# mantasu/face-crop-plus

Hardware: AMD Instinct MI355X
Metric: faces/sec end-to-end (detect+align+crop) (higher is better)
Workload: dtype f16x3; 1 GPU; RetinaFace detect + 5-pt align/crop, batch=32/GPU synthetic 1024x1024 RGB, strategy=largest, det_threshold=0.6, output 256x256, detector on 2 HIP streams x 16 images; global_batch=32, image_size=1024, parallelism=dp1

## Files before the change

### face-crop-plus_amd/csrc/fcp_bneck_chain.hip

```cpp
#include "fcp_conv_common.h"

#include <type_traits>

using namespace fcp_conv;

namespace {

constexpr int FCP_CHAIN_STORE_AUX = 2;

struct ChainK {
  const float* t1;  unsigned t1_bytes;  int t1_ld;
  const float* w2;  unsigned w2_bytes;  const float* ws2;  const float* b2;
  const float* w3;  unsigned w3_bytes;  const float* ws3;  const float* b3;
  const float* res; int res_ld;
  float* out;       int out_ld;    unsigned out_bytes;
  const float* w1n; unsigned w1n_bytes; const float* ws1n; const float* b1n;
  float* t1n;       int t1n_ld;
  int n, h, w, M;
  int nt_store;
  int out_even;
  const float* t1b; unsigned t1b_bytes; int t1b_ld, hb, wb, sb;
};

constexpr int BMT = 128;
constexpr int C = 64;
constexpr int ROWB = 128;
constexpr int STAGE = (BMT + C) * ROWB;
constexpr int CT_OFF = 0;
constexpr int W1B_OFF = BMT * 128;
constexpr bool w1_double(int cn, bool has_c2) { return !has_c2 || W1B_OFF + 2 * cn * 128 + 2 * C * 128 <= 2 * STAGE; }
constexpr int w3b_off(int cn, bool has_c2) { return W1B_OFF + (w1_double(cn, has_c2) ? 2 : 1) * cn * 128; }
constexpr int r0_bytes(int cw, int cn, bool has_c2) { return has_c2 ? 2 * STAGE : w3b_off(cn, has_c2) + 2 * cw * 128; }
constexpr bool alias_t2(bool has_c2) { return !has_c2; }
constexpr int lds_bytes(int cw, int cn, bool has_c2, bool direct = false) {
  const int r0 = r0_bytes(cw, cn, has_c2), t2 = BMT * cw * 4;
  if (direct) return r0;
  return !alias_t2(has_c2) ? r0 + t2 : (r0 > W1B_OFF + t2 ? r0 : W1B_OFF + t2);
}
constexpr int wgs_per_cu(int cw, int cn, bool has_c2, bool direct = false) {
  if (direct) return cn == 0 && lds_bytes(cw, cn, has_c2, true) <= 80 * 1024 ? 2 : 1;
  return lds_bytes(cw, cn, has_c2) <= 80 * 1024 ? 2 : 1;
}

__device__ __forceinline__ void mfma3(f32x16& acc, const f16x8& ah, const f16x8& al, const f16x8& bh, const f16x8& bl) {
  acc = __builtin_amdgcn_mfma_f32_32x32x16_f16(al, bh, acc, 0, 0, 0);
  acc = __builtin_amdgcn_mfma_f32_32x32x16_f16(ah, bl, acc, 0, 0, 0);
  acc = __builtin_amdgcn_mfma_f32_32x32x16_f16(ah, bh, acc, 0, 0, 0);
}

__device__ __forceinline__ void row_values8(const float* c8, const float (&ws8)[8], const float (&b8)[8], float (&v)[8]) {
  const f32x4 a = *reinterpret_cast<const f32x4*>(c8);
  const f32x4 b = *reinterpret_cast<const f32x4*>(c8 + 4);
#pragma unroll
  for (int e = 0; e < 4; ++e) {
    v[e] = conv_value_relu(a[e], ws8[e], b8[e]);
    v[4 + e] = conv_value_relu(b[e], ws8[4 + e], b8[4 + e]);
  }
}

constexpr bool direct_form(int cn, int cw2) { return cw2 > 0 || cn == 0; }
template <int CN, int CW, int NOUT, bool HAS_C2, bool HAS_RES, int CW2 = 0>
__global__ void __launch_bounds__(2 * BMT, wgs_per_cu(CW, CN, HAS_C2, direct_form(CN, CW2))) bneck_chain_c64(const ChainK p) {
  constexpr bool DIRECT = direct_form(CN, CW2);
  static_assert(!DIRECT || (!HAS_C2 && CW2 % 32 == 0 && CW2 < CW), "direct forms are pair forms");
  constexpr bool HAS_P3 = CN > 0;
  static_assert(!HAS_C2 || CW == C, "phase 1 is written for 64-channel bottlenecks");
  constexpr bool PATCH = HAS_C2;
  constexpr int PH = BMT / 16;
  constexpr int NTHR = 2 * BMT;
  constexpr int NW = NTHR / 64;
  constexpr int LR = NTHR / 8;
  constexpr int TN3 = CN / 32;
  constexpr int TN3A = TN3 > 0 ? TN3 : 1;
  constexpr int CS = CW / 32;
  constexpr int NCH = NOUT / 32;
  constexpr int W3CH = CW * 128;
  constexpr bool ALIAS = alias_t2(HAS_C2) && !DIRECT;
  constexpr int T2_OFF = ALIAS ? W1B_OFF : r0_bytes(CW, CN, HAS_C2);
  constexpr int WGS = wgs_per_cu(CW, CN, HAS_C2, DIRECT);
  constexpr int WPS = WGS * NW / 4;
  static_assert(lds_bytes(CW, CN, HAS_C2, DIRECT) <= 160 * 1024, "LDS budget");
  constexpr bool W1DB = w1_double(CN, HAS_C2);
  constexpr bool SPREAD = W1DB && (HAS_C2 || WPS == 1);
  constexpr bool W1PRE = W1DB && !DIRECT && (HAS_C2 ? CN <= 64 || WPS == 1 : CN <= 128 && WPS == 1);
  constexpr int W3B_OFF = w3b_off(CN, HAS_C2);
  static_assert(!HAS_C2 || W3B_OFF + 2 * W3CH <= 2 * STAGE, "chunk buffers must fit the phase-1 stage region");
  constexpr int NRES = HAS_RES ? 4 : 0;
  extern __shared__ __attribute__((aligned(16))) float smem[];
  char* lds = reinterpret_cast<char*>(smem);

  const int tile_m = xcd_tile_order(gridDim.x, blockIdx.x);

  const int tid = threadIdx.x;
  const int lane = tid & 63;
  const int wave = tid >> 6;
  const int wave_u = __builtin_amdgcn_readfirstlane(wave);
  const int lrow = tid >> 3;
  const int csrc = (tid & 7) ^ swz(lrow);
  const int l31 = lane & 31, half = lane >> 5;
  int offH[2], offL[2];
  frag_offsets(lane, offH, offL);
  auto frag_pair = [&](const char* row, int s, f16x8& hi, f16x8& lo) {
    hi = *reinterpret_cast<const f16x8*>(row + offH[s]);
    lo = *reinterpret_cast<const f16x8*>(row + offL[s]);
  };
  const int hw = p.h * p.w;
  int pn = 0, py0 = 0, px0 = 0;
  if constexpr (PATCH) {
    const int txn = (p.w + 15) >> 4, tyn = (p.h + PH - 1) / PH;
    const int r = tile_m / txn;
    px0 = (tile_m - r * txn) * 16;
    pn = r / tyn;
    py0 = (r - pn * tyn) * PH;
  }
  auto pix = [&](int row) -> long {
    if constexpr (PATCH) {
      const int y = py0 + (row >> 4), x = px0 + (row & 15);
      return (y < p.h && x < p.w) ? ((long)pn * p.h + y) * p.w + x : -1L;
    } else {
// ... 6 lines not shown
    float* Cs = smem;
#pragma unroll
    for (int i = 0; i < 2; ++i)
#pragma unroll
      for (int rr = 0; rr < 16; ++rr) {
        const int row = wm * 64 + i * 32 + (rr & 3) + 8 * (rr >> 2) + 4 * half;
        Cs[row * C + wn * 32 + l31] = acc1[i][rr];
      }
    __syncthreads();
    {
      const int ccol = (tid & 7) * 8;
      float ws8[8], b8[8];
#pragma unroll
      for (int e = 0; e < 8; ++e) {
        ws8[e] = p.ws2[ccol + e];
        b8[e] = p.b2[ccol + e];
      }
#pragma unroll
      for (int g = 0; g < 4; ++g) {
        const int row = (tid >> 3) + LR * g;
        float v[8];
        row_values8(Cs + row * C + ccol, ws8, b8, v);
        u32x4_t hi, lo;
        split8(f32x4{v[0], v[1], v[2], v[3]}, f32x4{v[4], v[5], v[6], v[7]}, hi, lo);
        const int q = (ccol & 31) >> 3, sw = swz(row);
        char* trow = lds + T2_OFF + (ccol >> 5) * (BMT * ROWB) + row * ROWB;
        *reinterpret_cast<u32x4_t*>(trow + ((q ^ sw) << 4)) = hi;
        *reinterpret_cast<u32x4_t*>(trow + (((4 + q) ^ sw) << 4)) = lo;
      }
    }
    __syncthreads();
  };

  if constexpr (HAS_C2) {
    constexpr int HALO = (PH + 2) * 18;
    constexpr int HROWS = (HALO + LR - 1) / LR * LR;
    constexpr int ASL = HROWS * ROWB;
    constexpr int TPB = 2, NSTEP = 18 / TPB;
    static_assert(18 % TPB == 0, "taps per barrier must divide the 18 K slices");
    constexpr int BST_OFF = 2 * ASL, BSL = C * ROWB, BSTG = TPB * BSL;
    static_assert(BST_OFF + 2 * BSTG <= T2_OFF + BMT * C * 4, "halo patch + filter stages must fit region 0 + T2");
    f32x16 acc1[2];
    const int wm = wave / 2, wn = wave % 2;
    __amdgpu_buffer_rsrc_t rs_in = __builtin_amdgcn_make_buffer_rsrc(const_cast<float*>(p.t1), 0, p.t1_bytes, 0x00020000);
    __amdgpu_buffer_rsrc_t rs_w = __builtin_amdgcn_make_buffer_rsrc(const_cast<float*>(p.w2), 0, p.w2_bytes, 0x00020000);
#pragma unroll
    for (int i = 0; i < HROWS / LR; ++i) {
      const int r = lrow + LR * i;
      const int hy = r / 18, hx = r - hy * 18;
      const int y = py0 - 1 + hy, x = px0 - 1 + hx;
      const bool ok = r < HALO && (unsigned)y < (unsigned)p.h && (unsigned)x < (unsigned)p.w;
      const unsigned src = ok ? ((unsigned)((pn * p.h + y) * p.w + x) * (unsigned)p.t1_ld + (unsigned)(csrc * 4)) * 4u : 0xFFFFFFFFu;
#pragma unroll
      for (int cs = 0; cs < 2; ++cs)
        __builtin_amdgcn_raw_ptr_buffer_load_lds(rs_in, (__attribute__((address_space(3))) void*)(lds + cs * ASL + (wave_u * 8 + LR * i) * ROWB), 16,
                                                 (int)(src == 0xFFFFFFFFu ? 0xFFFFFFFFu : src + (unsigned)(cs * 32 * 4)), 0, 0, 0);
    }
    constexpr int B_LD = C / LR;
    unsigned woff[B_LD];
#pragma unroll
    for (int i = 0; i < B_LD; ++i) woff[i] = (unsigned)(((lrow + LR * i) * (9 * C) + csrc * 4) * 4);
    auto dma_b = [&](int step, int stage) {
#pragma unroll
      for (int u = 0; u < TPB; ++u)
#pragma unroll
        for (int i = 0; i < B_LD; ++i)
          __builtin_amdgcn_raw_ptr_buffer_load_lds(rs_w, (__attribute__((address_space(3))) void*)(lds + BST_OFF + stage * BSTG + u * BSL + (wave_u * 8 + LR * i) * ROWB), 16,
                                                   (int)(woff[i] + (unsigned)((step * TPB + u) * BK * 4)), 0, 0, 0);
    };
    dma_b(0, 0);
#pragma unroll
    for (int i = 0; i < 2; ++i)
#pragma unroll
      for (int e = 0; e < 16; ++e) acc1[i][e] = 0.f;
    int hr0[2];
#pragma unroll
    for (int i = 0; i < 2; ++i) hr0[i] = (wm * 4 + i * 2 + (l31 >> 4)) * 18 + (l31 & 15);
    const char* Bw = lds + BST_OFF + (wn * 32 + l31) * ROWB;
    fcp_static_for<0, NSTEP>([&](auto gc) {
      constexpr int g = decltype(gc)::value;
      asm volatile("s_waitcnt vmcnt(0)" ::: "memory");
      __builtin_amdgcn_s_barrier();
      __builtin_amdgcn_sched_barrier(0);
      fcp_static_for<0, TPB>([&](auto uc) {
        constexpr int kt = g * TPB + decltype(uc)::value, cs = kt / 9, tap = kt % 9;
        const char* Bb = Bw + (g & 1) * BSTG + decltype(uc)::value * BSL;
        f16x8 ah[2][2], al[2][2], bh[2], bl[2];
#pragma unroll
        for (int i = 0; i < 2; ++i) {
          const int hr = hr0[i] + (tap / 3) * 18 + tap % 3;
          const int sw = swz(hr);
          const char* Ab = lds + cs * ASL + hr * ROWB;
#pragma unroll
          for (int sq = 0; sq < 2; ++sq) {
            ah[sq][i] = *reinterpret_cast<const f16x8*>(Ab + (((2 * sq + half) ^ sw) << 4));
            al[sq][i] = *reinterpret_cast<const f16x8*>(Ab + (((4 + 2 * sq + half) ^ sw) << 4));
          }
        }
#pragma unroll
        for (int sq = 0; sq < 2; ++sq) {
          frag_pair(Bb, sq, bh[sq], bl[sq]);
        }
        if constexpr (decltype(uc)::value == TPB - 1) {
// ... 67 lines not shown

  const char* a2base = lds + T2_OFF + (wave * 32 + l31) * ROWB;
  const char* a3base = lds + CT_OFF + (wave * 32 + l31) * ROWB;
  const int eq = lane & 3;
  const int erow0 = wave * 32 + (lane >> 2);
  long rm[2];
  unsigned so[2];
#pragma unroll
  for (int it = 0; it < 2; ++it) {
    const int prow = erow0 + 16 * it;
    const long m = pix(prow);
    rm[it] = m >= 0 ? m : (long)p.M - 1;
    const bool keep = !PATCH || !p.out_even || ((((prow >> 4) | prow) & 1) == 0);
    so[it] = (m >= 0 && keep) ? (unsigned)(m * p.out_ld * 4 + eq * 16) : 0xFFFFFFFFu;
  }
  __amdgpu_buffer_rsrc_t rs_out = __builtin_amdgcn_make_buffer_rsrc(p.out, 0, p.out_bytes, 0x00020000);

  u32x4_t rhi[2], rlo[2];
  auto load_res = [&](int j) {
    if constexpr (!HAS_RES) return;
#pragma unroll
    for (int it = 0; it < 2; ++it) {
      const char* pb = reinterpret_cast<const char*>(p.res) + rm[it] * p.res_ld * 4 + j * 128 + eq * 16;
      rhi[it] = *reinterpret_cast<const u32x4_t*>(pb);
      rlo[it] = *reinterpret_cast<const u32x4_t*>(pb + 64);
    }
  };
  const int nch = NCH;
  float ws_l = p.ws3[l31], b_l = p.b3[l31];
  constexpr int NCONST = 2;
  f16x8 ah[CS][2], al[CS][2];
  auto read_a2 = [&]() {
#pragma unroll
    for (int sl = 0; sl < CS; ++sl)
#pragma unroll
      for (int s = 0; s < 2; ++s) {
        frag_pair(a2base + sl * BMT * ROWB, s, ah[sl][s], al[sl][s]);
      }
  };
  if constexpr (DIRECT) {
    constexpr int CS1 = (CW - CW2) / 32;
    __amdgpu_buffer_rsrc_t rs_a = __builtin_amdgcn_make_buffer_rsrc(const_cast<float*>(p.t1), 0, p.t1_bytes, 0x00020000);
    __amdgpu_buffer_rsrc_t rs_b = __builtin_amdgcn_make_buffer_rsrc(const_cast<float*>(p.t1b), 0, p.t1b_bytes, 0x00020000);
    asm volatile("" ::: "memory");
    dma_w3(0, 0);
    if constexpr (W1DB) dma_w1(0, 0);
    asm volatile("" ::: "memory");
    const long m = pix(wave * 32 + l31);
    unsigned oa = 0xFFFFFFFFu, ob = 0xFFFFFFFFu;
    if (m >= 0) {
      const int ni = (int)(m / hw);
      const int rem = (int)(m - (long)ni * hw);
      const int y = rem / p.w, x = rem - y * p.w;
      oa = (unsigned)m * (unsigned)p.t1_ld * 4u;
      ob = ((unsigned)(ni * p.hb + y * p.sb) * (unsigned)p.wb + (unsigned)(x * p.sb)) * (unsigned)p.t1b_ld * 4u;
    }
#pragma unroll
    for (int sl = 0; sl < CS; ++sl)
#pragma unroll
      for (int sk = 0; sk < 2; ++sk) {
        const bool first = sl < CS1;
        const unsigned base = first ? oa : ob;
        const unsigned off = (unsigned)((first ? sl : sl - CS1) * 128);
        const unsigned vh = base == 0xFFFFFFFFu ? base : base + off + (unsigned)((2 * sk + half) << 4);
        const unsigned vl = base == 0xFFFFFFFFu ? base : base + off + (unsigned)((4 + 2 * sk + half) << 4);
        ah[sl][sk] = __builtin_bit_cast(f16x8, __builtin_amdgcn_raw_buffer_load_b128(first ? rs_a : rs_b, (int)vh, 0, 0));
        al[sl][sk] = __builtin_bit_cast(f16x8, __builtin_amdgcn_raw_buffer_load_b128(first ? rs_a : rs_b, (int)vl, 0, 0));
      }
    asm volatile("s_waitcnt vmcnt(0)" ::: "memory");
#pragma unroll
    for (int sl = 0; sl < CS; ++sl)
#pragma unroll
      for (int sk = 0; sk < 2; ++sk) asm volatile("" : "+v"(ah[sl][sk]), "+v"(al[sl][sk]));
    __builtin_amdgcn_sched_barrier(0);
  }
  if constexpr (ALIAS) {
    asm volatile("s_waitcnt vmcnt(0)" ::: "memory");
    __builtin_amdgcn_s_barrier();
    __builtin_amdgcn_sched_barrier(0);
    read_a2();
    asm volatile("s_waitcnt lgkmcnt(0)" ::: "memory");
    __builtin_amdgcn_s_barrier();
    __builtin_amdgcn_sched_barrier(0);
  }
  asm volatile("" ::: "memory");
  if constexpr (!DIRECT) {
    dma_w3(0, 0);
    if constexpr (W1DB) dma_w1(0, 0);
  }
  asm volatile("" ::: "memory");
  if (nch > 0) load_res(0);
  __builtin_amdgcn_sched_barrier(0);

  for (int j = 0; j < nch; ++j) {
    const bool more = j + 1 < NCH;
    if (j == 0) asm volatile("s_waitcnt vmcnt(%0)" ::"n"(NRES) : "memory");
    else asm volatile("s_waitcnt vmcnt(%0)" ::"n"(4 + NCONST + NRES) : "memory");
    asm volatile("s_waitcnt lgkmcnt(0)" ::: "memory");
    __builtin_amdgcn_s_barrier();
    __builtin_amdgcn_sched_barrier(0);
    if constexpr (!SPREAD) {
      if (more) dma_w3(j + 1, (j + 1) & 1);
      if constexpr (W1DB) {
        if (more) dma_w1(j + 1, (j + 1) & 1);
      } else {
        dma_w1(j, 0);
      }
    }
    asm volatile("" ::: "memory");
    __builtin_amdgcn_sched_barrier(0);
    const char* b2base = lds + W3B_OFF + (j & 1) * W3CH + l31 * ROWB;
    if constexpr (!ALIAS && !DIRECT) {
      if (j == 0) read_a2();
    }
    constexpr int BG = (CS <= 4 && (HAS_C2 || WPS == 1)) ? CS : 2;
    f16x8 bh[2][BG][2], bl[2][BG][2];
    auto read_b2 = [&](int buf, int g) {
#pragma unroll
      for (int q = 0; q < BG; ++q)
#pragma unroll
        for (int s = 0; s < 2; ++s) {
          frag_pair(b2base + (g * BG + q) * 4096, s, bh[buf][q][s], bl[buf][q][s]);
        }
    };
    read_b2(0, 0);
    f16x8 dh[2][TN3A], dl[2][TN3A];
    if constexpr (W1PRE) {
      const char* w1b = lds + W1B_OFF + (j & 1) * (CN * ROWB);
#pragma unroll
      for (int s = 0; s < 2; ++s)
#pragma unroll
        for (int t = 0; t < TN3; ++t) {
          frag_pair(w1b + (t * 32 + l31) * ROWB, s, dh[s][t], dl[s][t]);
        }
      __builtin_amdgcn_sched_barrier(0);
    }
    f32x16 acc2;
#pragma unroll
    for (int e = 0; e < 16; ++e) acc2[e] = 0.f;
    fcp_static_for<0, CS / BG>([&](auto gc) {
      constexpr int g = decltype(gc)::value;
      if constexpr (g + 1 < CS / BG) read_b2((g + 1) & 1, g + 1);
      fcp_static_for<0, 2 * BG>([&](auto tc) {
        constexpr int q = decltype(tc)::value / 2, s = decltype(tc)::value % 2, sl = g * BG + q, trip = 2 * sl + s;
        mfma3(acc2, ah[sl][s], al[sl][s], bh[g & 1][q][s], bl[g & 1][q][s]);
        constexpr int PER = (NDMA + 2 * CS - 1) / (2 * CS);
        if constexpr (SPREAD && trip * PER < NDMA) {
          __builtin_amdgcn_sched_barrier(0);
// ... 99 lines not shown
#pragma unroll
  for (int hh = 0; hh < CN / 64; ++hh) {
#pragma unroll
    for (int t = 0; t < 2; ++t)
#pragma unroll
      for (int rr = 0; rr < 16; ++rr) {
        const int row = wave * 32 + (rr & 3) + 8 * (rr >> 2) + 4 * half;
        Cs[row * 64 + t * 32 + l31] = acc3[CN == 64 ? t : 2 * hh + t][rr];
      }
    __syncthreads();
    const int ccol = (tid & 7) * 8;
    const int co = hh * 64 + ccol;
    float ws8[8], b8[8];
#pragma unroll
    for (int e = 0; e < 8; ++e) {
      ws8[e] = p.ws1n[co + e];
      b8[e] = p.b1n[co + e];
    }
#pragma unroll
    for (int g = 0; g < 4; ++g) {
      const int row = (tid >> 3) + LR * g;
      const long m = pix(row);
      if (m < 0) continue;
      float v[8];
      row_values8(Cs + row * 64 + ccol, ws8, b8, v);
      pack_store8(p.t1n, m, p.t1n_ld, co, 1, p.nt_store, v);
    }
    __syncthreads();
  }
}

template <int CN, int CW, int NOUT, bool HAS_C2, bool HAS_RES, int CW2 = 0>
int launch(const ChainK& k, hipStream_t s) {
  constexpr int LDS = lds_bytes(CW, CN, HAS_C2, direct_form(CN, CW2));
  FCP_LDS_OPT_IN((&bneck_chain_c64<CN, CW, NOUT, HAS_C2, HAS_RES, CW2>), LDS);
  const int tiles = HAS_C2 ? k.n * fcp_cdiv(k.h, BMT / 16) * ((k.w + 15) >> 4) : fcp_cdiv(k.M, BMT);
  hipLaunchKernelGGL((bneck_chain_c64<CN, CW, NOUT, HAS_C2, HAS_RES, CW2>), dim3(tiles), dim3(2 * BMT), LDS, s, k);
  FCP_LAUNCH_OK();
  return 0;
}

struct ChainForm {
  bool has_c2;
  int c, cb, nout;
  bool residual;
  int cn;
  int (*launch)(const ChainK&, hipStream_t);
};
const ChainForm FORMS[] = {
    {true, 64, 0, 256, true, 64, launch<64, 64, 256, true, true>},
    {true, 64, 0, 256, true, 128, launch<128, 64, 256, true, true>},
    {false, 128, 0, 512, true, 128, launch<128, 128, 512, false, true>},
    {false, 128, 0, 256, false, 64, launch<64, 128, 256, false, false>},
    {false, 256, 0, 1024, true, 256, launch<256, 256, 1024, false, true>},
    {false, 128, 0, 512, true, 256, launch<256, 128, 512, false, true>},
    {false, 384, 256, 512, false, 128, launch<128, 384, 512, false, false, 256>},
    {false, 256, 0, 1024, true, 0, launch<0, 256, 1024, false, true>},
};

}

extern "C" int fcp_bottleneck_chain_f16x3(const fcp_chain_desc* d, fcp_stream_t stream) {
  FCP_REQUIRE(d != nullptr, "chain: null descriptor");
  const bool has_p3 = d->cn != 0 || d->w1n != nullptr;
  FCP_REQUIRE(d->t1 && d->w3 && d->ws3 && d->b3 && d->out && (!has_p3 || (d->w1n && d->ws1n && d->b1n && d->t1n)),
              "chain: null pointer (every convolution carries folded-BN bias and filter scales)");
  const bool has_c2 = d->w2 != nullptr;
  FCP_REQUIRE(!has_c2 || (d->ws2 && d->b2), "chain: conv2 needs its scales and bias");
  const int cb = d->t1b ? d->cb : 0;
  const ChainForm* form = nullptr;
  for (const ChainForm& f : FORMS)
    if (f.has_c2 == has_c2 && f.c == d->c && f.cb == cb && f.nout == d->nout && f.residual == (d->res != nullptr) && f.cn == d->cn &&
        (f.cn != 0) == has_p3)
      form = &f;
  FCP_REQUIRE((form && form->cb) || !d->t1b, "chain: a second source (t1b) exists for the two-source pair form only (c 384 = 128 + 256, nout 512, cn 128)");
  FCP_REQUIRE(form != nullptr, "chain: unsupported shape (c %d, conv2 %d, nout %d, residual %d, cn %d)", d->c, (int)has_c2, d->nout,
              d->res != nullptr, d->cn);
  FCP_REQUIRE(d->n > 0 && d->h > 0 && d->w > 0, "chain: bad sizes");
  const long M = (long)d->n * d->h * d->w;
  FCP_REQUIRE(M < (1L << 31), "chain: too many pixels");
  auto aligned = [](const void* p, int ld) { return ((uintptr_t)p & 127) == 0 && ld % 32 == 0; };
  FCP_REQUIRE(aligned(d->t1, d->t1_ld) && (!d->res || aligned(d->res, d->res_ld)) && aligned(d->out, d->out_ld) && (!has_p3 || aligned(d->t1n, d->t1n_ld)),
              "chain: tensors are split32 views: 128-byte aligned, channel stride a multiple of 32");
  FCP_REQUIRE(d->t1_ld >= d->c - cb && (!d->res || d->res_ld >= d->nout) && d->out_ld >= d->nout && (!has_p3 || d->t1n_ld >= d->cn), "chain: channel strides too small");
  const unsigned long t1_bytes = (unsigned long)M * d->t1_ld * 4ul;
  FCP_REQUIRE(t1_bytes < 0xFFFFFFF0ul, "chain: t1 must be below 4 GiB");
  ChainK k;
  k.t1 = d->t1; k.t1_bytes = (unsigned)t1_bytes; k.t1_ld = d->t1_ld;
  k.w2 = reinterpret_cast<const float*>(d->w2); k.w2_bytes = 128u * 9 * 64 * 4; k.ws2 = d->ws2; k.b2 = d->b2;
  k.w3 = reinterpret_cast<const float*>(d->w3); k.w3_bytes = (unsigned)(d->nout * d->c * 4); k.ws3 = d->ws3; k.b3 = d->b3;
  k.res = d->res; k.res_ld = d->res_ld; k.out = d->out; k.out_ld = d->out_ld;
  const unsigned long out_bytes = (unsigned long)M * d->out_ld * 4ul;
  FCP_REQUIRE(out_bytes < 0xFFFFFFF0ul, "chain: out must span less than 4 GiB");
  k.out_bytes = (unsigned)out_bytes;
  k.w1n = reinterpret_cast<const float*>(d->w1n); k.w1n_bytes = has_p3 ? (unsigned)(fcp_cdiv(d->cn, 128) * 128 * d->nout * 4) : 0u; k.ws1n = d->ws1n; k.b1n = d->b1n;
  k.t1n = d->t1n; k.t1n_ld = d->t1n_ld;
  k.n = d->n; k.h = d->h; k.w = d->w; k.M = (int)M;
  static const int nt_env = getenv("FCP_NT_STORE") ? atoi(getenv("FCP_NT_STORE")) : 1;
  k.nt_store = nt_env;
  k.t1b = nullptr; k.t1b_bytes = 0; k.t1b_ld = 0; k.hb = 0; k.wb = 0; k.sb = 1;
  if (d->t1b) {
    FCP_REQUIRE(aligned(d->t1b, d->t1b_ld) && d->t1b_ld >= d->cb && d->t1b_stride >= 1 && d->t1b_h > 0 && d->t1b_w > 0 &&
                (long)(d->h - 1) * d->t1b_stride < d->t1b_h && (long)(d->w - 1) * d->t1b_stride < d->t1b_w,
                "chain: t1b must be a split32 view whose (h, w) grid covers the output grid at t1b_stride");
    const unsigned long tb = (unsigned long)d->n * d->t1b_h * d->t1b_w * d->t1b_ld * 4ul;
    FCP_REQUIRE(tb < 0xFFFFFFF0ul, "chain: t1b must be below 4 GiB");
    k.t1b = d->t1b; k.t1b_bytes = (unsigned)tb; k.t1b_ld = d->t1b_ld; k.hb = d->t1b_h; k.wb = d->t1b_w; k.sb = d->t1b_stride;
  }
  k.out_even = (d->flags & FCP_CHAIN_OUT_EVEN_ONLY) ? 1 : 0;
  FCP_REQUIRE(!k.out_even || has_c2, "chain: FCP_CHAIN_OUT_EVEN_ONLY needs a conv2 form");
  hipStream_t s = (hipStream_t)stream;
  return form->launch(k, s);
}
```

### face-crop-plus_amd/engine.py

```python
from __future__ import annotations

import contextlib
import ctypes as C
import os
import threading
from dataclasses import dataclass

import numpy as np
import torch

from . import _native as N
from . import torch_ops as T

BN_EPS = 1e-5
COUT_PAD = 128


class Act:
    __slots__ = ("buf", "c0", "c", "fmt")

    def __init__(self, buf: torch.Tensor, c0: int = 0, c: int | None = None, fmt: int = 0):
        assert buf.dim() == 4 and buf.dtype == torch.float32 and buf.is_contiguous()
        self.buf, self.c0, self.fmt = buf, c0, fmt
        self.c = buf.shape[3] - c0 if c is None else c
# ... 627 lines not shown
        byts = 4 * (m * (pc.cout + (pc.cout if res1 is not None else 0) + (pc.cout if res2 is not None else 0))
                    + x.n * in_h * in_w * x.c // (4 if in_up2 else 1) + (m * x2.c if x2 is not None else 0)
                    + pc.cout * pc.cin * pc.kh * pc.kw)
        head = f"conv {pc.kh}x{pc.kw} s{pc.stride} {pc.cin}->{pc.cout} @{oh}x{ow}"
        return (f"{head} tile {tm}x{tn}{' bal' if flags & N.CONV_BALANCE_TAIL else ''}{' +res' if res1 is not None else ''}",
                head, pc.flops_per_pixel * m, byts)

    def relaunch(o):
        o = _alias_safe_out(o, x, x2, res1, res2)
        return "fcp_conv2d_nhwc_f32", (C.byref(desc(o)),), (pc, x, x2, res1, res2, o)
    return _accounted(go, describe, relaunch)[0]


def tile_candidates(cout: int, halo_ok: bool, wide_ok: bool, big_ok: bool):
    cands = [(128, 128), (128, 64)]
    if halo_ok:
        cands = ([(128, 32)] if cout <= 32 else []) + [(128, 64), (1, 32)]
    if wide_ok:
        cands = cands + [(1, 128)]
    if big_ok:
        big = [(256, 128)] + ([(256, 256)] if cout >= 256 else []) + ([(256, 192)] if 128 < cout <= 192 else [])
        cands += big
        cands += [(tm, tn, N.CONV_BALANCE_TAIL) for tm, tn in big]
    return cands


def chain_supported(pc2: PackedConv | None, pc3: PackedConv, pc1n: PackedConv | None, residual: bool = True, cb: int = 0) -> bool:
    convs = [pc for pc in (pc2, pc3, pc1n) if pc is not None]
    if not all(pc.precision == 1 and pc.bias is not None and not pc.cin4 for pc in convs):
        return False
    one = lambda pc, cin, cout: (pc.cin, pc.cout, pc.kh, pc.kw, pc.stride, pc.pad) == (cin, cout, 1, 1, 1, 0)
    if pc1n is None:
        return pc2 is None and residual and not cb and one(pc3, 256, 1024)
    if cb:
        return pc2 is None and not residual and cb == 256 and one(pc3, 384, 512) and one(pc1n, 512, 128)
    if pc2 is not None:
        return ((pc2.cin, pc2.cout, pc2.kh, pc2.kw, pc2.stride, pc2.pad) == (64, 64, 3, 3, 1, 1) and residual
                and one(pc3, 64, 256) and (one(pc1n, 256, 64) or one(pc1n, 256, 128)))
    if residual:
        return ((one(pc3, 128, 512) and (one(pc1n, 512, 128) or one(pc1n, 512, 256)))
                or (one(pc3, 256, 1024) and one(pc1n, 1024, 256)))
    return one(pc3, 128, 256) and one(pc1n, 256, 64)



def _chain_desc(pc2, pc3, pc1n, t1, res, out, t1n, tile_m, flags, t1b, t1b_stride) -> N.ChainDesc:
    d = N.ChainDesc()
    d.t1, d.res, d.out = t1.ptr(), (res.ptr() if res is not None else None), out.ptr()
    d.t1n = t1n.ptr() if t1n is not None else None
    d.w2, d.ws2, d.b2 = map(N.ptr, _filter(pc2))
    d.w3, d.ws3, d.b3 = map(N.ptr, _filter(pc3))
    d.w1n, d.ws1n, d.b1n = map(N.ptr, _filter(pc1n))
    d.n, d.h, d.w, d.c, d.nout = t1.n, t1.h, t1.w, pc3.cin, pc3.cout
    d.cn = pc1n.cout if pc1n is not None else 0
    d.t1_ld, d.res_ld, d.out_ld = t1.ld, (res.ld if res is not None else 0), out.ld
    d.t1n_ld = t1n.ld if t1n is not None else 0
    d.tile_m, d.flags = tile_m, flags
    if t1b is not None:
        d.t1b, d.cb, d.t1b_ld, d.t1b_h, d.t1b_w, d.t1b_stride = t1b.ptr(), t1b.c, t1b.ld, t1b.h, t1b.w, t1b_stride
    return d


def bottleneck_chain(pc2: PackedConv | None, pc3: PackedConv, pc1n: PackedConv, t1: Act, res: Act | None,
                     out: Act | None = None, t1n: Act | None = None, tile_m: int = 0, out_even_only: bool = False,
                     t1b: Act | None = None, t1b_stride: int = 1):
    cb = t1b.c if t1b is not None else 0
    assert chain_supported(pc2, pc3, pc1n, res is not None, cb), "bottleneck_chain: unsupported shapes"
    assert t1.fmt == 1 and t1.c + cb == pc3.cin and (res is None or (res.fmt == 1 and res.c == pc3.cout))
    assert t1b is None or (t1b.fmt == 1 and t1b.n == t1.n and (t1.h - 1) * t1b_stride < t1b.h and (t1.w - 1) * t1b_stride < t1b.w)
    assert res is None or (t1.n, t1.h, t1.w) == (res.n, res.h, res.w)
    c, nout, cn = pc3.cin, pc3.cout, (pc1n.cout if pc1n is not None else 0)
    flags = N.CHAIN_OUT_EVEN_ONLY if (out_even_only and pc2 is not None and RangeMonitor.active is None) else 0
    via_op = T.ENABLED and out is None and t1n is None
    if not via_op:
        if out is None:
            out = Act.empty(t1.n, t1.h, t1.w, nout, t1.buf.device, 1)
        if t1n is None and pc1n is not None:
            t1n = Act.empty(t1.n, t1.h, t1.w, cn, t1.buf.device, 1)
        assert out.fmt == 1 and (out.n, out.h, out.w, out.c) == (t1.n, t1.h, t1.w, nout)
        assert pc1n is None or (t1n.fmt == 1 and (t1n.n, t1n.h, t1n.w, t1n.c) == (t1.n, t1.h, t1.w, cn))
    desc = lambda o, o1n: _chain_desc(pc2, pc3, pc1n, t1, res, o, o1n, tile_m, flags, t1b, t1b_stride)

    def go():
        if not via_op:
            _c_launch("fcp_bottleneck_chain_f16x3", C.byref(desc(out, t1n)))
            return out, t1n
        o, t = T.load().bottleneck_chain(t1.buf, t1.c0, None if res is None else res.buf, 0 if res is None else res.c0,
                                         *_filter(pc2), *_filter(pc3), *_filter(pc1n), c, nout, cn, tile_m, flags,
                                         None if t1b is None else t1b.buf, 0 if t1b is None else t1b.c0, cb, int(t1b_stride))
        return Act(o, fmt=1), (Act(t, fmt=1) if pc1n is not None else None)

    def describe():
        m = t1.n * t1.h * t1.w
        flops = ((pc2.flops_per_pixel if pc2 is not None else 0) + pc3.flops_per_pixel
                 + (pc1n.flops_per_pixel if pc1n is not None else 0)) * m
        byts = 4 * (m * (c + (nout if not flags else nout // 4) + (nout if res is not None else 0) + cn) + (0 if pc2 is None else 9 * c * c)
                    + c * nout + nout * cn)
        if pc1n is None:
            head = f"expand {c}->{nout} @{t1.h}x{t1.w}"
            return f"{head} +res", head, flops, byts
        head = f"chain {'3x3 ' if pc2 is not None else ''}{c}->{nout}->{cn} @{t1.h}x{t1.w}"
        return (f"{head}{' +res' if res is not None else ''}{' out@even' if flags else ''}{' two-source' if t1b is not None else ''}",
                head, flops, byts)

    def relaunch(o, o1n):
        o = _alias_safe_out(o, t1, res, t1b)
        o1n = o1n if o1n is None else _alias_safe_out(o1n, t1, res, t1b)
        return "fcp_bottleneck_chain_f16x3", (C.byref(desc(o, o1n)),), (pc2, pc3, pc1n, t1, res, o, o1n, t1b)
    return _accounted(go, describe, relaunch)


def u8_to_nhwc4(images_u8: torch.Tensor, sub=(0.0, 0.0, 0.0), div: float = 1.0) -> Act:
    assert images_u8.dtype == torch.uint8 and images_u8.dim() == 4 and images_u8.shape[3] == 3
    assert images_u8.is_contiguous()
    n, h, w, _ = images_u8.shape
    out = Act.empty(n, h, w, 4, images_u8.device)
    sub_arr = (C.c_float * 3)(*[float(s) for s in sub])
    N.check(N.lib().fcp_u8_to_nhwc4_f32(N.ptr(images_u8), out.ptr(), n * h * w, sub_arr, float(div),
                                        N.stream_ptr()), "fcp_u8_to_nhwc4_f32")
    return out


@dataclass
class PackedStem:
    wfrag: torch.Tensor
    bias: torch.Tensor
    wscale: torch.Tensor
    flops_per_pixel: int


def pack_stem_fused(weight, bn, device, cin_perm=None) -> PackedStem:
    if isinstance(weight, torch.Tensor):
        weight = weight.detach().cpu().numpy()
    bn = {k: (v.detach().cpu().numpy() if isinstance(v, torch.Tensor) else np.asarray(v)) for k, v in bn.items()}
    w, b = fold_bn(weight, bn, None)
    if cin_perm is not None:
        w = w[:, cin_perm]
    assert w.shape == (64, 3, 7, 7), "the fused stem is the ResNet 7x7 / 64-filter stem"
    wk = np.zeros((64, 22 * 8), np.float32)
    wk.reshape(64, 22, 8)
    for kh in range(7):
        wk[:, kh * 24:kh * 24 + 21] = w[:, :, kh, :].transpose(0, 2, 1).reshape(64, 21)
# ... 121 lines not shown
```

### face-crop-plus_amd/retinaface.py

```python
from __future__ import annotations


import os
import threading

import numpy as np
import torch

from . import _native as N
from . import engine as E
from . import torch_ops as T
from .weights import load_state_dict

STRATEGIES = {"all": 0, "best": 1, "largest": 2}


class RetinaFace:
    WEIGHTS_FILENAME = "retinaface_detector.pth"

    def __init__(self, strategy: str = "all", vis: float = 0.6):
        self.strategy = strategy
        self.vis_threshold = vis
        self.nms_threshold = 0.4
        self.variance = [0.1, 0.2]
# ... 82 lines not shown
                                   stride, 0, dev)
                    if stride == 1 or E.DEFAULT_PRECISION == 1:
                        fold = lambda cw, cb: E.fold_bn(sd[pre + cw].numpy(), {q: v.numpy() for q, v in bn(sd, pre + cb).items()}, None)
                        (w3, b3), (wd, bd) = fold(".conv3.weight", ".bn3"), fold(".downsample.0.weight", ".downsample.1")
                        blk["c3ds"] = pc(np.concatenate([w3, wd], 1), b3 + bd, None, 1, 0, dev)
                blocks.append(blk)
        p["blocks"] = blocks
        for i in (1, 2, 3):
            p[f"fpn.output{i}"] = pc(sd[f"fpn.output{i}.0.weight"], None, bn(sd, f"fpn.output{i}.1"), 1, 0, dev)
        for i in (1, 2):
            p[f"fpn.merge{i}"] = pc(sd[f"fpn.merge{i}.0.weight"], None, bn(sd, f"fpn.merge{i}.1"), 1, 1, dev)
        head_perm = list(range(0, 128)) + list(range(192, 256)) + list(range(128, 192))
        for k in (1, 2, 3):
            def folded(nm):
                return E.fold_bn(sd[f"ssh{k}.{nm}.0.weight"].numpy(), {q: v.numpy() for q, v in bn(sd, f"ssh{k}.{nm}.1").items()}, None)
            w_b, b_b = folded("conv5X5_1")
            w_a, b_a = folded("conv3X3")
            p[f"ssh{k}.ab"] = pc(np.concatenate([w_b, w_a]), np.concatenate([b_b, b_a]), None, 1, 1, dev)
            w_c, b_c = folded("conv5X5_2")
            w_d, b_d = folded("conv7X7_2")
            p[f"ssh{k}.cd"] = pc(np.concatenate([w_c, w_d]), np.concatenate([b_c, b_d]), None, 1, 1, dev)
            w_e, b_e = folded("conv7x7_3")
            p[f"ssh{k}.e"] = pc(w_e, b_e, None, 1, 1, dev)
            i = k - 1
            hw = np.concatenate([sd[f"{h}.{i}.conv1x1.weight"].numpy() for h in ("ClassHead", "BboxHead", "LandmarkHead")])
            hb = np.concatenate([sd[f"{h}.{i}.conv1x1.bias"].numpy() for h in ("ClassHead", "BboxHead", "LandmarkHead")])
            p[f"head{k}"] = pc(hw, hb, None, 1, 0, dev, cin_perm=head_perm)
        return p

    def forward_heads(self, x4: E.Act | None, images_u8: torch.Tensor | None = None, heads_out=None):
        p = self._p
        f = 1 if self.precision == 1 else 0
        stem_t1 = None
        if images_u8 is not None and "stem_fused" in p:
            n, h, w, _ = images_u8.shape
            hp, wp = ((h - 1) // 2) // 2 + 1, ((w - 1) // 2) // 2 + 1
            cat = E.Act.empty(n, hp, wp, 128, images_u8.device, f)
            c1 = p["blocks"][0]["c1"]
            if f == 1 and E.stem_conv1_supported(c1):
                x, stem_t1 = E.stem_relu_pool_u8(p["stem_fused"], images_u8, cat.slice(64, 64), conv1=c1)
            else:
                x = E.stem_relu_pool_u8(p["stem_fused"], images_u8, cat.slice(64, 64))
        else:
            x = E.conv(p["stem"], x4, act_slope=0.0, out_fmt=f)
            cat = E.Act.empty(x.n, (x.h + 1) // 2, (x.w + 1) // 2, 2 * x.c, x.buf.device, f)
            x = E.maxpool3x3s2(x, cat.slice(x.c, x.c))
        feats = []
        blocks, pre = p["blocks"], stem_t1
        chain = bool(f) and self.fused_chain
        for bi, blk in enumerate(blocks):
            o = pre if pre is not None else E.conv(blk["c1"], x, act_slope=0.0, out_fmt=f)
            pre = None
            nxt = blocks[bi + 1] if bi + 1 < len(blocks) else None
            if (chain and blk["ds"] is None and not blk["feat"] and nxt is not None
                    and E.chain_supported(blk["c2"], blk["c3"], nxt["c1"])):
                sparse = "c3ds" in nxt and nxt["c2"].stride == 2 and not blk["feat"]
                x, pre = E.bottleneck_chain(blk["c2"], blk["c3"], nxt["c1"], o, x, out_even_only=sparse)
                continue
            if "c3ds" in blk and blk["c2"].stride == 1:
                E.conv(blk["c2"], o, cat.slice(0, o.c), act_slope=0.0)
                if chain and nxt is not None and E.chain_supported(None, blk["c3ds"], nxt["c1"], residual=False):
                    x, pre = E.bottleneck_chain(None, blk["c3ds"], nxt["c1"], cat, None)
                else:
                    x = E.conv(blk["c3ds"], cat, act_slope=0.0, out_fmt=f)
                del cat
                continue
            if "c3ds" in blk:
                o = E.conv(blk["c2"], o, act_slope=0.0, out_fmt=f)
                if (chain and not blk["feat"] and nxt is not None
                        and E.chain_supported(None, blk["c3ds"], nxt["c1"], residual=False, cb=x.c)):
                    x, pre = E.bottleneck_chain(None, blk["c3ds"], nxt["c1"], o, None, t1b=x, t1b_stride=blk["c2"].stride)
                    continue
                x = E.conv(blk["c3ds"], o, act_slope=0.0, out_fmt=f, x2=x, x2_stride=blk["c2"].stride)
                if blk["feat"]:
                    feats.append(x)
                continue
            o = E.conv(blk["c2"], o, act_slope=0.0, out_fmt=f)
            if (chain and blk["ds"] is None and nxt is not None and E.chain_supported(None, blk["c3"], nxt["c1"])):
                x, pre = E.bottleneck_chain(None, blk["c3"], nxt["c1"], o, x)
                if blk["feat"]:
                    feats.append(x)
                continue
            idt = x if blk["ds"] is None else E.conv(blk["ds"], x, out_fmt=f)
            x = E.conv(blk["c3"], o, act_slope=0.0, res1=idt, res1_pre=True, out_fmt=f)
            if blk["feat"]:
                feats.append(x)
        if getattr(self, "_debug_feats", None) is not None:
            self._debug_feats.extend(feats)
        o3 = E.conv(p["fpn.output3"], feats[2], act_slope=0.0, out_fmt=f)
        o2 = E.conv(p["fpn.output2"], feats[1], act_slope=0.0, res1=o3, res1_pre=False, out_fmt=f)
# ... 197 lines not shown
```

Measured before the change: 1456 faces/s.

## Fuse layer1.0 conv2 with concatenated downsample expand into two-source chain kernel

Adds a two-source conv2 form to the bottleneck chain kernel for layer1.0. The 3x3 conv2 result and the pooled stem input, loaded directly from global memory into registers, feed the fused 128->256 expand and the next block's 1x1 conv. Before, conv2 was a separate launch writing into a concatenated buffer. The fusion removes that launch and the round trip of the 64-channel intermediate through HBM. In exchange it adds register pressure, a tighter LDS layout, and more template complexity.

Result: no change. 1463 faces/s (median of 6 runs) (+0.4%).

```diff
diff --git a/face-crop-plus_amd/csrc/fcp_bneck_chain.hip b/face-crop-plus_amd/csrc/fcp_bneck_chain.hip
--- a/face-crop-plus_amd/csrc/fcp_bneck_chain.hip
+++ b/face-crop-plus_amd/csrc/fcp_bneck_chain.hip
@@ -28,12 +28,15 @@
 constexpr int STAGE = (BMT + C) * ROWB;
 constexpr int CT_OFF = 0;
 constexpr int W1B_OFF = BMT * 128;
-constexpr bool w1_double(int cn, bool has_c2) { return !has_c2 || W1B_OFF + 2 * cn * 128 + 2 * C * 128 <= 2 * STAGE; }
-constexpr int w3b_off(int cn, bool has_c2) { return W1B_OFF + (w1_double(cn, has_c2) ? 2 : 1) * cn * 128; }
+constexpr bool two_source_c2(int cw, bool has_c2) { return has_c2 && cw > C; }
+constexpr bool w1_double(int cn, bool has_c2, int cw = C) {
+  return !has_c2 || W1B_OFF + 2 * cn * 128 + 2 * cw * 128 <= (two_source_c2(cw, has_c2) ? 2 * STAGE + BMT * C * 4 : 2 * STAGE);
+}
+constexpr int w3b_off(int cn, bool has_c2, int cw = C) { return W1B_OFF + (w1_double(cn, has_c2, cw) ? 2 : 1) * cn * 128; }
 constexpr int r0_bytes(int cw, int cn, bool has_c2) { return has_c2 ? 2 * STAGE : w3b_off(cn, has_c2) + 2 * cw * 128; }
 constexpr bool alias_t2(bool has_c2) { return !has_c2; }
 constexpr int lds_bytes(int cw, int cn, bool has_c2, bool direct = false) {
-  const int r0 = r0_bytes(cw, cn, has_c2), t2 = BMT * cw * 4;
+  const int r0 = r0_bytes(cw, cn, has_c2), t2 = BMT * (has_c2 ? C : cw) * 4;
   if (direct) return r0;
   return !alias_t2(has_c2) ? r0 + t2 : (r0 > W1B_OFF + t2 ? r0 : W1B_OFF + t2);
 }
@@ -58,13 +61,16 @@
   }
 }
 
-constexpr bool direct_form(int cn, int cw2) { return cw2 > 0 || cn == 0; }
+constexpr bool direct_form(int cn, int cw2, bool has_c2 = false) { return !has_c2 && (cw2 > 0 || cn == 0); }
 template <int CN, int CW, int NOUT, bool HAS_C2, bool HAS_RES, int CW2 = 0>
-__global__ void __launch_bounds__(2 * BMT, wgs_per_cu(CW, CN, HAS_C2, direct_form(CN, CW2))) bneck_chain_c64(const ChainK p) {
-  constexpr bool DIRECT = direct_form(CN, CW2);
+__global__ void __launch_bounds__(2 * BMT, wgs_per_cu(CW, CN, HAS_C2, direct_form(CN, CW2, HAS_C2))) bneck_chain_c64(const ChainK p) {
+  constexpr bool DIRECT = direct_form(CN, CW2, HAS_C2);
   static_assert(!DIRECT || (!HAS_C2 && CW2 % 32 == 0 && CW2 < CW), "direct forms are pair forms");
   constexpr bool HAS_P3 = CN > 0;
-  static_assert(!HAS_C2 || CW == C, "phase 1 is written for 64-channel bottlenecks");
+  static_assert(!HAS_C2 || CW == C + CW2, "phase 1 is written for 64-channel bottlenecks");
+  constexpr bool TWOSRC = HAS_C2 && CW2 > 0;
+  static_assert(!TWOSRC || (CW2 == 64 && !HAS_RES && two_source_c2(CW, HAS_C2)), "the two-source conv2 form is layer1.0's: 64 + 64 channels, no residual");
+  constexpr int CSL = HAS_C2 ? C / 32 : CW / 32;
   constexpr bool PATCH = HAS_C2;
   constexpr int PH = BMT / 16;
   constexpr int NTHR = 2 * BMT;
@@ -80,11 +86,13 @@
   constexpr int WGS = wgs_per_cu(CW, CN, HAS_C2, DIRECT);
   constexpr int WPS = WGS * NW / 4;
   static_assert(lds_bytes(CW, CN, HAS_C2, DIRECT) <= 160 * 1024, "LDS budget");
-  constexpr bool W1DB = w1_double(CN, HAS_C2);
+  constexpr bool W1DB = w1_double(CN, HAS_C2, CW);
   constexpr bool SPREAD = W1DB && (HAS_C2 || WPS == 1);
   constexpr bool W1PRE = W1DB && !DIRECT && (HAS_C2 ? CN <= 64 || WPS == 1 : CN <= 128 && WPS == 1);
-  constexpr int W3B_OFF = w3b_off(CN, HAS_C2);
-  static_assert(!HAS_C2 || W3B_OFF + 2 * W3CH <= 2 * STAGE, "chunk buffers must fit the phase-1 stage region");
+  constexpr int W3B_OFF = w3b_off(CN, HAS_C2, CW);
+  static_assert(!HAS_C2 || TWOSRC || W3B_OFF + 2 * W3CH <= 2 * STAGE, "chunk buffers must fit the phase-1 stage region");
+  static_assert(!TWOSRC || (W1DB && W3B_OFF + W3CH <= T2_OFF && W3B_OFF + 2 * W3CH <= lds_bytes(CW, CN, HAS_C2)),
+                "two-source conv2 form: the buffers filled before the chunk loop's first barrier lie below T2, the rest inside LDS");
   constexpr int NRES = HAS_RES ? 4 : 0;
   extern __shared__ __attribute__((aligned(16))) float smem[];
   char* lds = reinterpret_cast<char*>(smem);
@@ -157,6 +165,25 @@
     __syncthreads();
   };
 
+  constexpr int CSB = TWOSRC ? CW2 / 32 : 1;
+  f16x8 pbh[CSB][2], pbl[CSB][2];
+  auto load_second_source = [&]() {
+    __amdgpu_buffer_rsrc_t rs_b = __builtin_amdgcn_make_buffer_rsrc(const_cast<float*>(p.t1b), 0, p.t1b_bytes, 0x00020000);
+    const int row = wave * 32 + l31;
+    const int y = py0 + (row >> 4), x = px0 + (row & 15);
+    unsigned ob = (y < p.h && x < p.w) ? ((unsigned)((pn * p.hb + y * p.sb) * p.wb + x * p.sb) * (unsigned)p.t1b_ld) * 4u : 0xFFFFFFFFu;
+#pragma unroll
+    for (int sl = 0; sl < CSB; ++sl)
+#pragma unroll
+      for (int sk = 0; sk < 2; ++sk) {
+        unsigned vh = ob == 0xFFFFFFFFu ? ob : ob + (unsigned)(sl * 128 + ((2 * sk + half) << 4));
+        unsigned vl = ob == 0xFFFFFFFFu ? ob : ob + (unsigned)(sl * 128 + ((4 + 2 * sk + half) << 4));
+        asm volatile("" : "+v"(vh), "+v"(vl));
+        pbh[sl][sk] = __builtin_bit_cast(f16x8, __builtin_amdgcn_raw_buffer_load_b128(rs_b, (int)vh, 0, 0));
+        pbl[sl][sk] = __builtin_bit_cast(f16x8, __builtin_amdgcn_raw_buffer_load_b128(rs_b, (int)vl, 0, 0));
+      }
+  };
+
   if constexpr (HAS_C2) {
     constexpr int HALO = (PH + 2) * 18;
     constexpr int HROWS = (HALO + LR - 1) / LR * LR;
@@ -194,6 +221,11 @@
                                                    (int)(woff[i] + (unsigned)((step * TPB + u) * BK * 4)), 0, 0, 0);
     };
     dma_b(0, 0);
+    if constexpr (TWOSRC) {
+      asm volatile("" ::: "memory");
+      load_second_source();
+      asm volatile("" ::: "memory");
+    }
 #pragma unroll
     for (int i = 0; i < 2; ++i)
 #pragma unroll
@@ -327,7 +359,7 @@
   f16x8 ah[CS][2], al[CS][2];
   auto read_a2 = [&]() {
 #pragma unroll
-    for (int sl = 0; sl < CS; ++sl)
+    for (int sl = 0; sl < CSL; ++sl)
 #pragma unroll
       for (int s = 0; s < 2; ++s) {
         frag_pair(a2base + sl * BMT * ROWB, s, ah[sl][s], al[sl][s]);
@@ -378,6 +410,19 @@
     __builtin_amdgcn_s_barrier();
     __builtin_amdgcn_sched_barrier(0);
   }
+  if constexpr (TWOSRC) {
+#pragma unroll
+    for (int sl = 0; sl < CSB; ++sl)
+#pragma unroll
+      for (int sk = 0; sk < 2; ++sk) {
+        asm volatile("" : "+v"(pbh[sl][sk]), "+v"(pbl[sl][sk]));
+        ah[CSL + sl][sk] = pbh[sl][sk];
+        al[CSL + sl][sk] = pbl[sl][sk];
+      }
+    __builtin_amdgcn_sched_barrier(0);
+    read_a2();
+    __builtin_amdgcn_sched_barrier(0);
+  }
   asm volatile("" ::: "memory");
   if constexpr (!DIRECT) {
     dma_w3(0, 0);
@@ -386,6 +431,14 @@
   asm volatile("" ::: "memory");
   if (nch > 0) load_res(0);
   __builtin_amdgcn_sched_barrier(0);
+  if constexpr (TWOSRC) {
+    asm volatile("s_waitcnt lgkmcnt(0)" ::: "memory");
+#pragma unroll
+    for (int sl = 0; sl < CSL; ++sl)
+#pragma unroll
+      for (int sk = 0; sk < 2; ++sk) asm volatile("" : "+v"(ah[sl][sk]), "+v"(al[sl][sk]));
+    __builtin_amdgcn_sched_barrier(0);
+  }
 
   for (int j = 0; j < nch; ++j) {
     const bool more = j + 1 < NCH;
@@ -405,10 +458,10 @@
     asm volatile("" ::: "memory");
     __builtin_amdgcn_sched_barrier(0);
     const char* b2base = lds + W3B_OFF + (j & 1) * W3CH + l31 * ROWB;
-    if constexpr (!ALIAS && !DIRECT) {
+    if constexpr (!ALIAS && !DIRECT && !TWOSRC) {
       if (j == 0) read_a2();
     }
-    constexpr int BG = (CS <= 4 && (HAS_C2 || WPS == 1)) ? CS : 2;
+    constexpr int BG = TWOSRC ? 1 : (CS <= 4 && (HAS_C2 || WPS == 1)) ? CS : 2;
     f16x8 bh[2][BG][2], bl[2][BG][2];
     auto read_b2 = [&](int buf, int g) {
 #pragma unroll
@@ -574,7 +627,7 @@
 
 template <int CN, int CW, int NOUT, bool HAS_C2, bool HAS_RES, int CW2 = 0>
 int launch(const ChainK& k, hipStream_t s) {
-  constexpr int LDS = lds_bytes(CW, CN, HAS_C2, direct_form(CN, CW2));
+  constexpr int LDS = lds_bytes(CW, CN, HAS_C2, direct_form(CN, CW2, HAS_C2));
   FCP_LDS_OPT_IN((&bneck_chain_c64<CN, CW, NOUT, HAS_C2, HAS_RES, CW2>), LDS);
   const int tiles = HAS_C2 ? k.n * fcp_cdiv(k.h, BMT / 16) * ((k.w + 15) >> 4) : fcp_cdiv(k.M, BMT);
   hipLaunchKernelGGL((bneck_chain_c64<CN, CW, NOUT, HAS_C2, HAS_RES, CW2>), dim3(tiles), dim3(2 * BMT), LDS, s, k);
@@ -592,6 +645,7 @@
 const ChainForm FORMS[] = {
     {true, 64, 0, 256, true, 64, launch<64, 64, 256, true, true>},
     {true, 64, 0, 256, true, 128, launch<128, 64, 256, true, true>},
+    {true, 128, 64, 256, false, 64, launch<64, 128, 256, true, false, 64>},
     {false, 128, 0, 512, true, 128, launch<128, 128, 512, false, true>},
     {false, 128, 0, 256, false, 64, launch<64, 128, 256, false, false>},
     {false, 256, 0, 1024, true, 256, launch<256, 256, 1024, false, true>},
@@ -615,7 +669,9 @@
     if (f.has_c2 == has_c2 && f.c == d->c && f.cb == cb && f.nout == d->nout && f.residual == (d->res != nullptr) && f.cn == d->cn &&
         (f.cn != 0) == has_p3)
       form = &f;
-  FCP_REQUIRE((form && form->cb) || !d->t1b, "chain: a second source (t1b) exists for the two-source pair form only (c 384 = 128 + 256, nout 512, cn 128)");
+  FCP_REQUIRE((form && form->cb) || !d->t1b,
+              "chain: a second source (t1b) exists for the two-source pair form (c 384 = 128 + 256, nout 512, cn 128) and the two-source conv2 form "
+              "(conv2, c 128 = 64 + 64, nout 256, cn 64, t1b_stride 1) only");
   FCP_REQUIRE(form != nullptr, "chain: unsupported shape (c %d, conv2 %d, nout %d, residual %d, cn %d)", d->c, (int)has_c2, d->nout,
               d->res != nullptr, d->cn);
   FCP_REQUIRE(d->n > 0 && d->h > 0 && d->w > 0, "chain: bad sizes");
@@ -649,6 +705,7 @@
     FCP_REQUIRE(tb < 0xFFFFFFF0ul, "chain: t1b must be below 4 GiB");
     k.t1b = d->t1b; k.t1b_bytes = (unsigned)tb; k.t1b_ld = d->t1b_ld; k.hb = d->t1b_h; k.wb = d->t1b_w; k.sb = d->t1b_stride;
   }
+  FCP_REQUIRE(!(has_c2 && d->t1b) || d->t1b_stride == 1, "chain: the two-source conv2 form reads t1b at the output's own pixels (t1b_stride 1)");
   k.out_even = (d->flags & FCP_CHAIN_OUT_EVEN_ONLY) ? 1 : 0;
   FCP_REQUIRE(!k.out_even || has_c2, "chain: FCP_CHAIN_OUT_EVEN_ONLY needs a conv2 form");
   hipStream_t s = (hipStream_t)stream;
diff --git a/face-crop-plus_amd/engine.py b/face-crop-plus_amd/engine.py
--- a/face-crop-plus_amd/engine.py
+++ b/face-crop-plus_amd/engine.py
@@ -683,10 +683,13 @@
     one = lambda pc, cin, cout: (pc.cin, pc.cout, pc.kh, pc.kw, pc.stride, pc.pad) == (cin, cout, 1, 1, 1, 0)
     if pc1n is None:
         return pc2 is None and residual and not cb and one(pc3, 256, 1024)
+    c2_ok = pc2 is not None and (pc2.cin, pc2.cout, pc2.kh, pc2.kw, pc2.stride, pc2.pad) == (64, 64, 3, 3, 1, 1)
+    if cb and pc2 is not None:
+        return c2_ok and not residual and cb == 64 and one(pc3, 128, 256) and one(pc1n, 256, 64)
     if cb:
-        return pc2 is None and not residual and cb == 256 and one(pc3, 384, 512) and one(pc1n, 512, 128)
+        return not residual and cb == 256 and one(pc3, 384, 512) and one(pc1n, 512, 128)
     if pc2 is not None:
-        return ((pc2.cin, pc2.cout, pc2.kh, pc2.kw, pc2.stride, pc2.pad) == (64, 64, 3, 3, 1, 1) and residual
+        return (c2_ok and residual
                 and one(pc3, 64, 256) and (one(pc1n, 256, 64) or one(pc1n, 256, 128)))
     if residual:
         return ((one(pc3, 128, 512) and (one(pc1n, 512, 128) or one(pc1n, 512, 256)))
@@ -712,13 +715,14 @@
     return d
 
 
-def bottleneck_chain(pc2: PackedConv | None, pc3: PackedConv, pc1n: PackedConv, t1: Act, res: Act | None,
-                     out: Act | None = None, t1n: Act | None = None, tile_m: int = 0, out_even_only: bool = False,
-                     t1b: Act | None = None, t1b_stride: int = 1):
+def _chain_launch(pc2: PackedConv | None, pc3: PackedConv, pc1n: PackedConv, t1: Act, res: Act | None,
+                  out: Act | None = None, t1n: Act | None = None, tile_m: int = 0, out_even_only: bool = False,
+                  t1b: Act | None = None, t1b_stride: int = 1):
     cb = t1b.c if t1b is not None else 0
     assert chain_supported(pc2, pc3, pc1n, res is not None, cb), "bottleneck_chain: unsupported shapes"
     assert t1.fmt == 1 and t1.c + cb == pc3.cin and (res is None or (res.fmt == 1 and res.c == pc3.cout))
     assert t1b is None or (t1b.fmt == 1 and t1b.n == t1.n and (t1.h - 1) * t1b_stride < t1b.h and (t1.w - 1) * t1b_stride < t1b.w)
+    assert t1b is None or pc2 is None or t1b_stride == 1, "the two-source conv2 form reads t1b at the output's own pixels"
     assert res is None or (t1.n, t1.h, t1.w) == (res.n, res.h, res.w)
     c, nout, cn = pc3.cin, pc3.cout, (pc1n.cout if pc1n is not None else 0)
     flags = N.CHAIN_OUT_EVEN_ONLY if (out_even_only and pc2 is not None and RangeMonitor.active is None) else 0
@@ -745,12 +749,13 @@
         m = t1.n * t1.h * t1.w
         flops = ((pc2.flops_per_pixel if pc2 is not None else 0) + pc3.flops_per_pixel
                  + (pc1n.flops_per_pixel if pc1n is not None else 0)) * m
-        byts = 4 * (m * (c + (nout if not flags else nout // 4) + (nout if res is not None else 0) + cn) + (0 if pc2 is None else 9 * c * c)
+        byts = 4 * (m * (c + (nout if not flags else nout // 4) + (nout if res is not None else 0) + cn) + (0 if pc2 is None else 9 * pc2.cin * pc2.cout)
                     + c * nout + nout * cn)
         if pc1n is None:
             head = f"expand {c}->{nout} @{t1.h}x{t1.w}"
             return f"{head} +res", head, flops, byts
-        head = f"chain {'3x3 ' if pc2 is not None else ''}{c}->{nout}->{cn} @{t1.h}x{t1.w}"
+        cin = f"{c - cb}+{cb}" if (pc2 is not None and cb) else f"{c}"
+        head = f"chain {'3x3 ' if pc2 is not None else ''}{cin}->{nout}->{cn} @{t1.h}x{t1.w}"
         return (f"{head}{' +res' if res is not None else ''}{' out@even' if flags else ''}{' two-source' if t1b is not None else ''}",
                 head, flops, byts)
 
@@ -759,6 +764,17 @@
         o1n = o1n if o1n is None else _alias_safe_out(o1n, t1, res, t1b)
         return "fcp_bottleneck_chain_f16x3", (C.byref(desc(o, o1n)),), (pc2, pc3, pc1n, t1, res, o, o1n, t1b)
     return _accounted(go, describe, relaunch)
+
+
+def bottleneck_chain(pc2: PackedConv | None, pc3: PackedConv, pc1n: PackedConv, t1: Act, res: Act | None,
+                     out: Act | None = None, t1n: Act | None = None, tile_m: int = 0, out_even_only: bool = False,
+                     t1b: Act | None = None, t1b_stride: int = 1):
+    return _chain_launch(pc2, pc3, pc1n, t1, res, out, t1n, tile_m, out_even_only, t1b, t1b_stride)
+
+
+def bottleneck_chain_two_source(pc2: PackedConv, pc3: PackedConv, pc1n: PackedConv, t1: Act, t1b: Act,
+                                out: Act | None = None, t1n: Act | None = None):
+    return _chain_launch(pc2, pc3, pc1n, t1, None, out, t1n, t1b=t1b)
 
 
 def u8_to_nhwc4(images_u8: torch.Tensor, sub=(0.0, 0.0, 0.0), div: float = 1.0) -> Act:
diff --git a/face-crop-plus_amd/retinaface.py b/face-crop-plus_amd/retinaface.py
--- a/face-crop-plus_amd/retinaface.py
+++ b/face-crop-plus_amd/retinaface.py
@@ -138,22 +138,30 @@
         p = self._p
         f = 1 if self.precision == 1 else 0
         stem_t1 = None
+        blocks = p["blocks"]
+        chain = bool(f) and self.fused_chain
+        l10 = (chain and len(blocks) > 1 and "c3ds" in blocks[0] and blocks[0]["c2"].stride == 1
+               and E.chain_supported(blocks[0]["c2"], blocks[0]["c3ds"], blocks[1]["c1"], residual=False, cb=64))
+        def pool_views(n, hp, wp, c, dev):
+            if l10:
+                return None, E.Act.empty(n, hp, wp, c, dev, f)
+            cat = E.Act.empty(n, hp, wp, 2 * c, dev, f)
+            return cat, cat.slice(c, c)
         if images_u8 is not None and "stem_fused" in p:
             n, h, w, _ = images_u8.shape
             hp, wp = ((h - 1) // 2) // 2 + 1, ((w - 1) // 2) // 2 + 1
-            cat = E.Act.empty(n, hp, wp, 128, images_u8.device, f)
-            c1 = p["blocks"][0]["c1"]
+            cat, pv = pool_views(n, hp, wp, 64, images_u8.device)
+            c1 = blocks[0]["c1"]
             if f == 1 and E.stem_conv1_supported(c1):
-                x, stem_t1 = E.stem_relu_pool_u8(p["stem_fused"], images_u8, cat.slice(64, 64), conv1=c1)
+                x, stem_t1 = E.stem_relu_pool_u8(p["stem_fused"], images_u8, pv, conv1=c1)
             else:
-                x = E.stem_relu_pool_u8(p["stem_fused"], images_u8, cat.slice(64, 64))
+                x = E.stem_relu_pool_u8(p["stem_fused"], images_u8, pv)
         else:
             x = E.conv(p["stem"], x4, act_slope=0.0, out_fmt=f)
-            cat = E.Act.empty(x.n, (x.h + 1) // 2, (x.w + 1) // 2, 2 * x.c, x.buf.device, f)
-            x = E.maxpool3x3s2(x, cat.slice(x.c, x.c))
+            cat, pv = pool_views(x.n, (x.h + 1) // 2, (x.w + 1) // 2, x.c, x.buf.device)
+            x = E.maxpool3x3s2(x, pv)
         feats = []
-        blocks, pre = p["blocks"], stem_t1
-        chain = bool(f) and self.fused_chain
+        pre = stem_t1
         for bi, blk in enumerate(blocks):
             o = pre if pre is not None else E.conv(blk["c1"], x, act_slope=0.0, out_fmt=f)
             pre = None
@@ -162,6 +170,9 @@
                     and E.chain_supported(blk["c2"], blk["c3"], nxt["c1"])):
                 sparse = "c3ds" in nxt and nxt["c2"].stride == 2 and not blk["feat"]
                 x, pre = E.bottleneck_chain(blk["c2"], blk["c3"], nxt["c1"], o, x, out_even_only=sparse)
+                continue
+            if "c3ds" in blk and blk["c2"].stride == 1 and l10 and bi == 0:
+                x, pre = E.bottleneck_chain_two_source(blk["c2"], blk["c3ds"], nxt["c1"], o, x)
                 continue
             if "c3ds" in blk and blk["c2"].stride == 1:
                 E.conv(blk["c2"], o, cat.slice(0, o.c), act_slope=0.0)
```
